# FlowEternal/multitask-hydranet

Hardware: AMD Instinct MI355X
Metric: images/sec (fwd+bwd) HydraNet @ default res, 1/2/4/8 MI355X; CPU-ref same run (higher is better)
Workload: dtype bf16; 1 GPU; full HydraNet (backbone + BiFPN + seg/det/lane heads + multitask loss), big cfg, fwd+loss+bwd; batch_per_gpu=16, global_batch=16, resolution=3x512x1024, parallelism=dp1, hipgraph=True

## Files before the change

include/hydranet_hip.h:

```cpp
#ifndef HYDRANET_HIP_H
#define HYDRANET_HIP_H

#ifdef __cplusplus
extern "C" {
#endif

typedef struct ihipStream_t* hipStream_t;


int hn_gconv_pack_diag(const float* w, void* wk, void* wd, int C, hipStream_t stream);
int hn_pack_weight(const float* w, void* wp, void* wt, int Cout, int Cin, int taps, hipStream_t stream);
int hn_pack_weight_ex(const float* w, void* wp, void* wt, int Cout, int Cin_total, int ci0, int Cin, int taps, int phase, const float* bias,
                      float* b_eff, hipStream_t stream);
int hn_phase_fold(const float* dw_eff, const float* dw1, const float* db_eff, float* dw, float* db, int K, int C0, int C1, hipStream_t stream);
int hn_pack_weights_batched(const long* jobs, int njobs, long total_blocks, const int* block_job, hipStream_t stream);
int hn_pack_small_batched(const long* jobs, const int* block_job, long total_blocks, hipStream_t stream);

int hn_conv_gemm_nt(const void* x0, const void* x1, int mode, int n_img, int H, int W, int C0, int C1, int ld0, int ld1, int up, long M,
                    const void* w, int Nout, int KP, int taps, const float* bias, int act, void* out, int out_f32, int ldc, long rpi,
                    long img_stride, float* psum, float* psq, hipStream_t stream);
int hn_nt_stat_rows(long M, int Nout);
int hn_nt_stat_tile(long M, int Nout);
int hn_direct_stat_rows(int n_img, int H, int W);
int hn_conv_gemm_nt_imgw(const void* x0, int ld0, long M, int C0, const void* w, long w_img_stride, long rows_per_image, int Nout, int KP,
// ... 14 lines not shown
                         int ld_ez, const float* ecoef, hipStream_t stream);
int hn_conv_gemm_nt_stat3(const void* x0, int ld0, long M, int C0, const void* w, int Nout, int KP, void* out, int ldc, float* psum, float* psq,
                          const void* addend, int ld_add, const void* ez, int ld_ez, const void* ey, int ld_ey, const float* ecoef,
                          hipStream_t stream);
int hn_wgrad_plan(int mode, int n_img, int H, int W, long M, int Nout, int KP, int taps, int* splits, long* rows_per_split, long* ws_bytes);
int hn_conv_gemm_tn(const void* x0, const void* x1, int mode, int n_img, int H, int W, int C0, int C1, int ld0, int ld1, int up, long M,
                    const void* dz, int ldz, int Nout, int KP, int taps, float* workspace, float* dw, hipStream_t stream);


int hn_stem_fwd(const float* x, const float* w, void* z, void* patches, int N, int H, int W, hipStream_t stream);

int hn_gconv_pack(const float* w, void* wk, void* wd, int C, int flip, hipStream_t stream);
int hn_gconv_fwd(const void* in, int ldi, const void* wk, void* out, int ldo, int N, int Hi, int Wi, int C, int stride, hipStream_t stream);
int hn_gconv_dgrad_s2(const void* dz, int ldz, const void* wd, void* dx, int ldx, int N, int Hi, int Wi, int C, hipStream_t stream);
long hn_wgrad_chunks(long pixels, long items);
int hn_gconv_wgrad(const void* x, int ldx, const void* dz, int ldz, float* part, int N, int Hi, int Wi, int C, int stride,
                   hipStream_t stream);

int hn_dw_pack(const float* w, void* wk, void* wkf, int C, hipStream_t stream);
int hn_dwconv_fwd(const void* in, int ldi, const void* wk, void* out, int ldo, int N, int H, int W, int C, hipStream_t stream);
int hn_dwconv_fwd_levels(const void* in, int ldi, const void* wk, void* out, int ldo, int N, int C, int nlev, const int* H, const int* W,
                         int row_align, int accumulate, hipStream_t stream);
long hn_dwconv_wgrad_blocks(long strips, int C);
int hn_dwconv_wgrad(const void* x, int ldx, const void* dz, int ldz, float* part, int N, int H, int W, int C, hipStream_t stream);
int hn_dwconv_wgrad_levels(const void* x, int ldx, const void* dz, int ldz, float* part, int N, int C, int nlev, const int* H, const int* W,
                           int row_align, hipStream_t stream);
long hn_dwconv_bwd_blocks(long strips, int C);
long hn_dwconv_bwd_blocks_levels(int N, int C, int nlev, const int* H, const int* W);
int hn_dwconv_bwd_levels(const void* dz, int ldz, const void* x, int ldx, const void* wf, void* dx, int lddx, float* part, int N, int C,
                         int nlev, const int* H, const int* W, int row_align, int accumulate, hipStream_t stream);

int hn_maxpool_fwd(const void* in, int ldi, void* out, int ldo, int N, int H, int W, int C, int mode, hipStream_t stream);
int hn_maxpool_bwd(const void* in, int ldi, const void* dout, int ldd, void* dx, int ldx, const float* wscale, int N, int H, int W, int C,
                   int mode, hipStream_t stream);
int hn_maxpool_bwd2(const void* in, int ldi, const void* dout, int ldd, void* dx, int ldx, const float* wscale, void* arg_ws, int N, int H,
                    int W, int C, int mode, int accumulate, hipStream_t stream);

int hn_up2_fwd(const void* in, int ldi, void* out, int ldo, int N, int H, int W, int C, hipStream_t stream);
int hn_sum2x2(const void* g, int ldg, void* out, int ldo, const float* wscale, int N, int H, int W, int C, int accumulate, hipStream_t stream);

int hn_fuse_dweights(const float* pw, int blocks, const float* praw, int nw, float eps, float* dp, hipStream_t stream);
int hn_fuse_fwd(const void* const* in, const int* ld, const int* mode, const float* w, void* out, int ldo, int N, int H, int W, int C,
                hipStream_t stream);
int hn_fuse_fwd_raw(const void* const* in, const int* ld, const int* mode, const float* praw, int nw, float eps, float* wn, void* out, int ldo,
                    int N, int H, int W, int C, hipStream_t stream);
int hn_fuse_bwd_blocks(int N, int H, int W, int C);
int hn_fuse_bwd(const void* const* in, const int* ld, const int* mode, const float* w, const void* dout, int ldd, void* g, int ldg,
                void* const* din, const int* ldin, const int* acc, float* pw, int N, int H, int W, int C, hipStream_t stream);
int hn_fuse_bwd_arg(const void* const* in, const int* ld, const int* mode, const float* w, const void* dout, int ldd, void* g, int ldg,
                    void* const* din, const int* ldin, const int* acc, float* pw, void* const* arg_out, int N, int H, int W, int C,
                    hipStream_t stream);
int hn_maxpool_bwd_from_arg(const void* arg, const void* dout, int ldd, void* dx, int ldx, const float* wscale, int N, int H, int W, int C,
                            int mode, int accumulate, hipStream_t stream);

long hn_fold_ring_rows(int H, int W);
int hn_conv3x3_dgrad_fold(const void* dz, int ldz, int Cz, int n_img, int H, int W, const void* wt, int Nout, int KP, int phase_k, int clamp,
                          void* out, int ldo, const void* yprev, int ldy, void* ring, hipStream_t stream);
int hn_conv3x3_dgrad_fold_s2d(const void* dz, int ldz, int Cz, int n_img, int H, int W, const void* wt, int Nout, int KP, int phase_k, int clamp,
                              void* out, int ldo, void* out_s2d, int ld_s2d, const void* yprev, int ldy, void* ring, hipStream_t stream);
int hn_seg_fold(const void* dvp, int ldv, int c0, void* out, int ldo, const void* yprev, int ldy, int N, int H, int W, int C, int up,
                hipStream_t stream);

int hn_space_to_depth(const float* dy, void* out, int ldo, int N, int h, int w, int k, hipStream_t stream);

int hn_space_to_depth_blocks(int N, int h, int w, int k);
int hn_space_to_depth_bf16(const void* in, int ldi, void* out, int N, int h, int w, int k, float* psum, hipStream_t stream);

int hn_conv3x3_phase(const void* x0, int mode, int n_img, int H, int W, int C0, int ld0, const void* w, int Nout, int KP, const float* bias,
                     int act, void* out, int ldc, int k, const void* addend, int ld_add, hipStream_t stream);
int hn_conv3x3_out_argmax(const void* x0, int n_img, int H, int W, int C0, int ld0, const void* w, int k, int KP, const float* bias, long* mask,
                          hipStream_t stream);
int hn_wgrad_plan_phase(int n_img, int H, int W, int Nout, int KP, int phase_span, int* splits, long* rows_per_split, long* ws_bytes);
int hn_conv_gemm_tn_phase(const void* x0, int n_img, int H, int W, int C0, int ld0, const void* dz, int ldz, int Nout, int KP, int phase_span,
                          float* workspace, float* dw, float* dbias_eff, hipStream_t stream);
int hn_conv_gemm_tn_deferred(const void* x0, const void* x1, int mode, int n_img, int H, int W, int C0, int C1, int ld0, int ld1, int up, long M,
                             const void* dz, int ldz, int Nout, int KP, int taps, float* workspace, float* dw, long* job, hipStream_t stream);
int hn_wgrad_reduce_jobs(const long* jobs, int njobs, hipStream_t stream);
long hn_gconv_wgrad_group_ws_bytes(const long* jobs, int njobs);
int hn_gconv_wgrad_group(const long* jobs, int njobs, float* workspace, hipStream_t stream);

int hn_grad_tail(const long* jobs, int njobs, hipStream_t stream);

long hn_wgrad_group_ws_bytes(const long* jobs, int njobs);
int hn_wgrad_group(const long* jobs, int njobs, float* workspace, hipStream_t stream);

int hn_conv_gemm_tn_bias(const void* x0, const void* x1, int mode, int n_img, int H, int W, int C0, int C1, int ld0, int ld1, int up, long M,
                         const void* dz, int ldz, int Nout, int KP, int taps, float* workspace, float* dw, float* dbias, hipStream_t stream);

int hn_head_grad(const float* dy, const float* y, long rpi, long img_stride, int lds, int Nout, void* dz, int ldz, long M, int sigmoid,
                 hipStream_t stream);

int hn_pack_levels(const void* const* src, const int* ld, void* dst, int ldd, int N, int C, int nlev, const int* H, const int* W, int row_align,
                   hipStream_t stream);
int hn_head_grad_levels(const float* dy, const float* y, long img_stride, int lds, int Nout, void* dz, int ldz, int N, int nlev, const int* H,
                        const int* W, int row_align, int sigmoid, hipStream_t stream);


long hn_colred_rows(long M, long align);
int hn_col_stats(const void* x, int ldx, long M, int C, long R, float* psum, float* psq, hipStream_t stream);
int hn_col_dot(const void* a, int lda, const void* b, int ldb, long M, int C, long R, float* pdot, float* psum, hipStream_t stream);
int hn_rows_reduce(const float* in, float* out, int G, int S, int C, float alpha, hipStream_t stream);
int hn_rows_reduce2(const float* in1, const float* in2, float* out1, float* out2, int rows, int G, int C, hipStream_t stream);

int hn_bn_finalize(const float* psum, const float* psq, int prows, int C, long count, const float* gamma, const float* beta, float eps,
                   float momentum, float* running_mean, float* running_var, float* scale, float* shift, float* mean, float* rstd,
                   hipStream_t stream);
// ... 193 lines not shown
```

multitask_hydranet_amd/_lib.py:

```python
from __future__ import annotations

import ctypes
import os
import re
import subprocess
from typing import Dict, List, Tuple

_PKG = os.path.dirname(os.path.abspath(__file__))
_ROOT = os.path.dirname(_PKG)
HEADER = os.path.join(_ROOT, "include", "hydranet_hip.h")
CSRC = os.path.join(_PKG, "csrc")
TUNING = os.environ.get("HN_TUNING") == "1"
AB = TUNING or os.environ.get("HN_TUNING") == "ab"


def policy(name: str, default: str) -> str:
    return os.environ.get(name, default) if AB else default

SO_PATH = os.path.join(_PKG, "libhydranet_hip_tuning.so" if TUNING else "libhydranet_hip.so")
SOURCES = ["hn_gemm.hip", "hn_norm.hip", "hn_fused.hip", "hn_stencil.hip", "hn_loss.hip", "hn_lovasz.hip", "hn_post.hip", "hn_xstage.hip", "hn_coco.hip",
           "hn_lane_encode.hip", "hn_augment.hip", "hn_jpeg.hip", "hn_jpeg_enc.hip", "hn_jpeg_huff.hip", "hn_jpeg_scan.hip", "hn_draw.hip", "hn_lane_metric.hip", "hn_png.hip", "hn_png_enc.hip"]

_ERR = {1: "bad argument", 2: "kernel launch failure", 3: "unsupported shape"}


class HipKernelError(RuntimeError):
    pass


def _ctype(decl: str):
    decl = decl.strip()
    if "*" in decl or "hipStream_t" in decl:
        return ctypes.c_void_p
    words = decl.replace("const", " ").split()
    base = words[0]
    return {"int": ctypes.c_int, "long": ctypes.c_long, "float": ctypes.c_float, "double": ctypes.c_double}[base]


TUNING_HEADER = os.path.join(_ROOT, "include", "hydranet_hip_tuning.h")


def parse_header(path: str = HEADER) -> Dict[str, Tuple[object, List[object], bool]]:
    txt = open(path).read()
    if TUNING and path == HEADER:
        txt += open(TUNING_HEADER).read()
    txt = re.sub(r"/\*.*?\*/", " ", txt, flags=re.S)
    out = {}
    for m in re.finditer(r"\b(int|long)\s+(hn_\w+)\s*\((.*?)\)\s*;", txt, flags=re.S):
        ret, name, params = m.group(1), m.group(2), m.group(3)
        plist = [p for p in (q.strip() for q in params.replace("\n", " ").split(",")) if p and p != "void"]
        args = [_ctype(p) for p in plist]
        out[name] = (ctypes.c_int if ret == "int" else ctypes.c_long, args, bool(plist) and "hipStream_t" in plist[-1])
    return out


def sources() -> List[str]:
    return [os.path.join(CSRC, s) for s in SOURCES if os.path.exists(os.path.join(CSRC, s))]


def build(force: bool = False, verbose: bool = False) -> str:
    srcs = sources()
    deps = srcs + [os.path.join(CSRC, "hn_common.h"), os.path.join(CSRC, "hn_jpeg_tables.h"), os.path.join(CSRC, "hn_jpeg_scan.h")]
    if not force and os.path.exists(SO_PATH) and all(os.path.getmtime(SO_PATH) >= os.path.getmtime(d) for d in deps):
        return SO_PATH
    hipcc = os.environ.get("HIPCC", "/opt/rocm/bin/hipcc")
    objs = []
    procs = []
    for s in srcs:
        o = os.path.join(CSRC, os.path.basename(s).replace(".hip", ".tuning.o" if TUNING else ".o"))
        objs.append(o)
        cmd = [hipcc, "--offload-arch=gfx950", "-O3", "-fPIC", "-std=c++17"] + (["-DHN_TUNING"] if TUNING else []) + ["-c", s, "-o", o]
        if verbose:
            print(" ".join(cmd))
        procs.append((cmd, subprocess.Popen(cmd, stdout=subprocess.PIPE, stderr=subprocess.STDOUT)))
# ... 57 lines not shown
```

multitask_hydranet_amd/csrc/hn_common.h:

```cpp
#pragma once
#include <hip/hip_runtime.h>
#include <stdint.h>

typedef __bf16 bf16;
typedef bf16 bf16x4 __attribute__((ext_vector_type(4)));
typedef bf16 bf16x2 __attribute__((ext_vector_type(2)));
typedef bf16 bf16x8 __attribute__((ext_vector_type(8)));
typedef short short4v __attribute__((ext_vector_type(4)));
typedef float f32x4 __attribute__((ext_vector_type(4)));
typedef unsigned int u32x4 __attribute__((ext_vector_type(4)));
typedef unsigned int u32x2 __attribute__((ext_vector_type(2)));

#define HN_OK 0
#define HN_ERR_ARG 1
#define HN_ERR_LAUNCH 2
#define HN_ERR_UNSUPPORTED 3

#define HN_CHECK_ARG(cond) do { if (!(cond)) return HN_ERR_ARG; } while (0)
#define HN_LAUNCH_CHECK() do { if (hipGetLastError() != hipSuccess) return HN_ERR_LAUNCH; return HN_OK; } while (0)

__device__ __forceinline__ float bf2f(bf16 v) { return (float)v; }
__device__ __forceinline__ bf16 f2bf(float v) { return (bf16)v; }
__device__ __forceinline__ float bfround(float v) { return (float)((bf16)v); }

// ... 59 lines not shown
        for (int k = 0; k < N; ++k) v[k] = v[k] > 0.f ? v[k] : 0.f;
    } else if (act == HN_ACT_SWISH) {
#pragma unroll
        for (int k = 0; k < N; ++k) v[k] = v[k] * sigmoidf_(v[k]);
    } else if (act == HN_ACT_ELU) {
#pragma unroll
        for (int k = 0; k < N; ++k) v[k] = v[k] > 0.f ? v[k] : (__expf(v[k]) - 1.0f);
    } else {
#pragma unroll
        for (int k = 0; k < N; ++k) v[k] = sigmoidf_(v[k]);
    }
}
template <int N>
__device__ __forceinline__ void act_bwd_n(const float (&x)[N], float (&g)[N], int act) {
    if (act == HN_ACT_NONE) return;
    if (act == HN_ACT_RELU) {
#pragma unroll
        for (int k = 0; k < N; ++k) g[k] = x[k] > 0.f ? g[k] : 0.f;
    } else if (act == HN_ACT_SWISH) {
#pragma unroll
        for (int k = 0; k < N; ++k) { const float s = sigmoidf_(x[k]); g[k] *= s * (1.f + x[k] * (1.f - s)); }
    } else if (act == HN_ACT_ELU) {
#pragma unroll
        for (int k = 0; k < N; ++k) g[k] *= x[k] > 0.f ? 1.f : __expf(x[k]);
    } else {
#pragma unroll
        for (int k = 0; k < N; ++k) { const float s = sigmoidf_(x[k]); g[k] *= s * (1.f - s); }
    }
}

__device__ __forceinline__ int xcd_remap(int hw, int nwg) {
    const int q = nwg >> 3, r = nwg & 7, x = hw & 7;
    return (x < r ? x * (q + 1) : r * (q + 1) + (x - r) * q) + (hw >> 3);
}

template <int CTRL>
__device__ __forceinline__ float dpp_mov(float v) {
    return __builtin_bit_cast(float, __builtin_amdgcn_update_dpp(0, __builtin_bit_cast(int, v), CTRL, 0xf, 0xf, false));
}
__device__ __forceinline__ float row16_sum(float v) {
    v += dpp_mov<0x128>(v);
    v += dpp_mov<0x124>(v);
    v += dpp_mov<0x122>(v);
    v += dpp_mov<0x121>(v);
    return v;
}

__device__ __forceinline__ float wave_sum(float v) {
    const int b = __builtin_bit_cast(int, row16_sum(v));
    return (__builtin_bit_cast(float, __builtin_amdgcn_readlane(b, 0)) + __builtin_bit_cast(float, __builtin_amdgcn_readlane(b, 16))) +
           (__builtin_bit_cast(float, __builtin_amdgcn_readlane(b, 32)) + __builtin_bit_cast(float, __builtin_amdgcn_readlane(b, 48)));
}

static inline int cdiv(long a, long b) { return (int)((a + b - 1) / b); }

#include <atomic>
#include <initializer_list>
static inline bool lds_optin(std::atomic<unsigned long long>& done, std::initializer_list<const void*> kernels) {
    int dev = 0;
    if (hipGetDevice(&dev) != hipSuccess || dev < 0 || dev >= 64) return false;
    const unsigned long long bit = 1ull << dev;
    if (done.load(std::memory_order_acquire) & bit) return true;
    for (const void* k : kernels)
        if (hipFuncSetAttribute(k, hipFuncAttributeMaxDynamicSharedMemorySize, 160 * 1024) != hipSuccess) return false;
    done.fetch_or(bit, std::memory_order_release);
    return true;
}
```

multitask_hydranet_amd/csrc/hn_stencil.hip:

```cpp
#include "hn_common.h"

__global__ __launch_bounds__(256) void stem_fwd_kernel(const float* x, const float* w, bf16* z, bf16* patches, int N, int H, int W) {
    const int bidx = xcd_remap(blockIdx.x, gridDim.x);
    __shared__ float sw[27][32];
    for (int i = threadIdx.x; i < 27 * 32; i += 256) {
        const int co = i & 31, t = i >> 5;
        sw[t][co] = w[co * 27 + t];
    }
    __syncthreads();
    const int Ho = H >> 1, Wo = W >> 1, Wp = (Wo + 1) >> 1;
    const long total = (long)N * Ho * Wp;
    const long idx = (long)bidx * 256 + threadIdx.x;
    if (idx >= total) return;
    const int ox = (int)(idx % Wp) * 2;
    const long t1 = idx / Wp;
    const int oy = (int)(t1 % Ho);
    const long n = t1 / Ho;
    const bool two = ox + 1 < Wo;
    float acc[2][32];
#pragma unroll
    for (int c = 0; c < 32; ++c) { acc[0][c] = 0.f; acc[1][c] = 0.f; }
    __shared__ __attribute__((aligned(16))) bf16 sp[2][256][36];
    bf16* prow = patches ? sp[0][threadIdx.x] : nullptr;
    constexpr int PH = 256 * 36;
// ... 819 lines not shown
                    for (int j = 0; j < 3; ++j) {
                        const bf16x4 zq = win[(rq + rr) % 3][j];
#pragma unroll
                        for (int k = 0; k < 4; ++k) {
                            const float zf = bf2f(zq[k]);
                            if (HAS_DX) da[k] = fmaf(zf, wr[rr * 3 + j][k], da[k]);
                            acc[8 - (rr * 3 + j)][k] = fmaf(xv[k], zf, acc[8 - (rr * 3 + j)][k]);
                        }
                    }
                if (HAS_DX && oy0 + r < H && ox0 + col < W) {
                    bf16* dst = dx + (row0 + (long)(oy0 + r) * W + ox0 + col) * lddx + cq * 4;
                    bf16x4 v;
                    if (accumulate) {
                        const bf16x4 prev = ld4(dst);
#pragma unroll
                        for (int k = 0; k < 4; ++k) v[k] = f2bf(da[k] + bf2f(prev[k]));
                    } else {
#pragma unroll
                        for (int k = 0; k < 4; ++k) v[k] = f2bf(da[k]);
                    }
                    *reinterpret_cast<bf16x4*>(dst) = v;
                }
            }
        }
    }
    __syncthreads();
    float* red = reinterpret_cast<float*>(smem);
    if (active) {
#pragma unroll
        for (int tq = 0; tq < 9; ++tq)
#pragma unroll
            for (int k = 0; k < 4; ++k) red[(colh * C4 + cq) * 37 + tq * 4 + k] = acc[tq][k];
    }
    __syncthreads();
    float* dst = part + (long)bidx * C * 9;
    for (int o = tid; o < C4 * 36; o += 256) {
        const int g = o / 36, v = o - g * 36;
        float sum = 0.f;
#pragma unroll
        for (int c2 = 0; c2 < 8; ++c2) sum += red[(c2 * C4 + g) * 37 + v];
        dst[(long)(g * 4 + (v & 3)) * 9 + (v >> 2)] = sum;
    }
}

__global__ void dw_pack_kernel(const float* w, bf16* wk, bf16* wkf, int C) {
    const int idx = blockIdx.x * blockDim.x + threadIdx.x;
    if (idx >= 9 * C) return;
    const int c = idx % C, tap = idx / C;
    const bf16 v = f2bf(w[c * 9 + tap]);
    wk[idx] = v;
    if (wkf) wkf[(8 - tap) * C + c] = v;
}

__device__ __forceinline__ void pool_window(const bf16* in, int ldi, long n, int H, int W, int oy, int ox, int c, int mode, float* best,
                                            int* arg) {
#pragma unroll
    for (int k = 0; k < 8; ++k) { best[k] = -INFINITY; arg[k] = -1; }
    const int off = mode ? -1 : 0;
#pragma unroll
    for (int ky = 0; ky < 3; ++ky)
#pragma unroll
        for (int kx = 0; kx < 3; ++kx) {
            const int iy = 2 * oy + ky + off, ix = 2 * ox + kx + off;
            const bool inside = iy >= 0 && iy < H && ix >= 0 && ix < W;
            if (!inside && mode) continue;
            bf16x8 v = inside ? ld8(in + ((n * H + iy) * (long)W + ix) * ldi + c) : zero8();
#pragma unroll
            for (int k = 0; k < 8; ++k) {
                const float f = bf2f(v[k]);
                if (f > best[k]) { best[k] = f; arg[k] = inside ? ky * 3 + kx : 9; }
            }
        }
}

__global__ __launch_bounds__(256) void maxpool_fwd_kernel(const bf16* in, int ldi, bf16* out, int ldo, int N, int H, int W, int C,
                                                          int mode) {
    const int bidx = xcd_remap(blockIdx.x, gridDim.x);
    const int C8 = C >> 3, Ho = H >> 1, Wo = W >> 1;
    const long total = (long)N * Ho * Wo * C8;
    for (long idx = (long)bidx * 256 + threadIdx.x; idx < total; idx += (long)gridDim.x * 256) {
        const int cg = (int)(idx % C8);
        long t = idx / C8;
        const int ox = (int)(t % Wo);
        t /= Wo;
        const int oy = (int)(t % Ho);
        const long n = t / Ho;
        float best[8];
        int arg[8];
        pool_window(in, ldi, n, H, W, oy, ox, cg * 8, mode, best, arg);
        bf16x8 v;
#pragma unroll
        for (int k = 0; k < 8; ++k) v[k] = f2bf(best[k]);
        st8(out + ((n * Ho + oy) * (long)Wo + ox) * ldo + cg * 8, v);
    }
}

__global__ __launch_bounds__(256) void maxpool_bwd_kernel(const bf16* in, int ldi, const bf16* dout, int ldd, bf16* dx, int ldx,
                                                          const float* wscale, int N, int H, int W, int C, int mode) {
    const int bidx = xcd_remap(blockIdx.x, gridDim.x);
    const int C8 = C >> 3, Ho = H >> 1, Wo = W >> 1;
    const long total = (long)N * H * W * C8;
    const float ws = wscale ? *wscale : 1.0f;
    const int off = mode ? -1 : 0;
    for (long idx = (long)bidx * 256 + threadIdx.x; idx < total; idx += (long)gridDim.x * 256) {
        const int cg = (int)(idx % C8);
        long t = idx / C8;
        const int ix = (int)(t % W);
        t /= W;
        const int iy = (int)(t % H);
        const long n = t / H;
        float acc[8];
#pragma unroll
        for (int k = 0; k < 8; ++k) acc[k] = 0.f;
        for (int oy = (iy - off - 2 + 1) >> 1; 2 * oy + off <= iy; ++oy) {
            if (oy < 0 || oy >= Ho) continue;
            for (int ox = (ix - off - 2 + 1) >> 1; 2 * ox + off <= ix; ++ox) {
                if (ox < 0 || ox >= Wo) continue;
                float best[8];
                int arg[8];
                pool_window(in, ldi, n, H, W, oy, ox, cg * 8, mode, best, arg);
                const int mine = (iy - 2 * oy - off) * 3 + (ix - 2 * ox - off);
                const bf16x8 g = ld8(dout + ((n * Ho + oy) * (long)Wo + ox) * ldd + cg * 8);
#pragma unroll
                for (int k = 0; k < 8; ++k)
                    if (arg[k] == mine) acc[k] += bf2f(g[k]);
            }
        }
// ... 979 lines not shown
```

multitask_hydranet_amd/model.py:

```python
from __future__ import annotations

import contextlib
import itertools
import math
import sys
import weakref
from typing import Dict, List, Optional, Sequence

import numpy as np
import torch
import torch.nn as nn

from . import ops as K
from .ops import ACT_ELU, ACT_NONE, ACT_RELU, ACT_SIGMOID, ACT_SWISH

BN_STD = dict(eps=1e-5, momentum=0.1)
BN_FPN = dict(eps=1e-3, momentum=0.01)


def regnet_stages(initial_width, slope, quantized_param, network_depth, bottleneck_ratio, group_width):
    u = initial_width + slope * np.arange(network_depth)
    s = np.round(np.log(u / initial_width) / np.log(quantized_param))
    q = 8 * np.round(initial_width * np.power(quantized_param, s) / 8)
    widths, depths = np.unique(q.astype(np.int32), return_counts=True)
# ... 386 lines not shown
        x = x.contiguous().float()
        t = self._cba(x, p + "stem.conv", p + "stem.bn", BN_STD, kind="stem", act=ACT_RELU)
        feats = []
        P = self._idx
        for k, d in enumerate(self.depths):
            group = None
            names = [f"{p}stage_{k}.blocks.block_{i}.{c}" for i in range(d)
                     for c in ("conv_block_1.0.weight", "conv_block_2.0.weight", "conv_block_3.0.weight", "shortcut.0.weight", "se.1.weight",
                               "se.1.bias", "se.3.weight", "se.3.bias")]
            names = [nm for nm in names if nm in P]
            if (K.DEFER_WGRAD and self.training and torch.is_grad_enabled() and t.requires_grad and t.is_cuda and (self.se_ratio is not None) and
                    all(P[nm].requires_grad for nm in names)):
                group = K.WgradGroup()
                t = K.DeferredGrads.apply(t, group, *[P[nm] for nm in names])
            i = 0
            while i < d:
                q = f"{p}stage_{k}.blocks.block_{i}."
                if i > 0 and self.training and not (torch.is_grad_enabled() and t.requires_grad) and self._xstage_shape_ok(q, t):
                    while i < d:
                        j1 = min(d, i + 16)
                        params = []
                        for j in range(i, j1):
                            params += self._xblock_params(f"{p}stage_{k}.blocks.block_{j}.")
                        with torch.no_grad():
                            t = K.xstage_forward_raw(t, params, BN_STD["eps"], BN_STD["momentum"])["out"][j1 - i - 1]
                        i = j1
                    break
                if i > 0 and i < d and self._xstage_run(q, t, group):
                    while i < d:
                        j1 = min(d, i + 16)
                        params = []
                        for j in range(i, j1):
                            params += self._xblock_params(f"{p}stage_{k}.blocks.block_{j}.")
                        t = K.xstage_apply(t, group, BN_STD["eps"], BN_STD["momentum"], params)
                        i = j1
                    break
                t = self._xblock(q, t, self.backbone_stride if i == 0 else 1, group)
                i += 1
            last = k == len(self.depths) - 1
            if last and tail is not None and K.DEFER_WGRAD and self.training and torch.is_grad_enabled() and t.requires_grad and t.is_cuda:
                t = K.DeferredGrads.apply(t, tail[0], *tail[1])
                tail[2] = True
            al, slot = K.share(t, ext[k] + (0 if last else 1))
            feats.append((al[:ext[k]], slot))
            if not last:
                t = al[-1]
        return feats

    def _sepconv(self, name, x, act=ACT_NONE):
        P = self._idx
        d = K.DwConv.apply(x, P[name + ".depthwise_conv.conv.weight"])
        return self._cba(d, name + ".pointwise_conv.conv", name + ".bn", BN_FPN, act=act)

    def _fusew(self, name):
        return self._idx[name]

    CELL_IN_COUNTS = (1, 2, 2, 2, 2)

    def _cell_shared(self, p, inputs, first, ext):
        red = lambda nm, src, i: self._cba(src[0][i], p + nm + ".0.conv", p + nm + ".1", BN_FPN, act=ACT_NONE, slot=src[1])
        sh = K.share
        if first:
            if len(inputs) == 4:
                p3, p4, p5 = inputs[-3:]
                p6_in = K.MaxPool.apply(red("p5_to_p6", p5, 2), 0)
            else:
                p3, p4, p5, p6r = inputs[-4:]
                p6_in = red("p6_down_channel", p6r, 0)
            (p6a, p6b, p6c), s6 = sh(p6_in, 3)
            p7_in = K.MaxPool.apply(p6c, 0)
            p3a, s3 = red("p3_down_channel", p3, 0), None
            (p4a, p4b), s4a, s4b = (red("p4_down_channel", p4, 0), red("p4_down_channel_2", p4, 1)), None, None
            (p5a, p5b), s5a, s5b = (red("p5_down_channel", p5, 0), red("p5_down_channel_2", p5, 1)), None, None
        else:
            (p3a,), s3 = inputs[0]
            (p4a, p4b), s4a = inputs[1]
            (p5a, p5b), s5a = inputs[2]
            (p6a, p6b), s6 = inputs[3]
            s4b, s5b = s4a, s5a
        if first:
            (p7a, p7b), s7 = sh(p7_in, 2)
        else:
            (p7a, p7b), s7 = inputs[4]
        F = K.Fuse.apply
        w = lambda nm: self._fusew(p + nm)
        (u6a, u6b), t6 = sh(self._sepconv(p + "conv6_up", F(w("p6_w1"), 1, 2, 0, p6a, p7a, None, (s6, s7, None))), 2)
        (u5a, u5b), t5 = sh(self._sepconv(p + "conv5_up", F(w("p5_w1"), 1, 2, 0, p5a, u6a, None, (s5a, t6, None))), 2)
        (u4a, u4b), t4 = sh(self._sepconv(p + "conv4_up", F(w("p4_w1"), 1, 2, 0, p4a, u5a, None, (s4a, t5, None))), 2)
        o3, q3 = sh(self._sepconv(p + "conv3_up", F(w("p3_w1"), 1, 2, 0, p3a, u4a, None, (s3, t4, None))), 1 + ext[0])
        o4, q4 = sh(self._sepconv(p + "conv4_down", F(w("p4_w2"), 1, 1, 3, p4b, u4b, o3[0], (s4b, t4, q3))), 1 + ext[1])
        o5, q5 = sh(self._sepconv(p + "conv5_down", F(w("p5_w2"), 1, 1, 3, p5b, u5b, o4[0], (s5b, t5, q4))), 1 + ext[2])
        o6, q6 = sh(self._sepconv(p + "conv6_down", F(w("p6_w2"), 1, 1, 3, p6b, u6b, o5[0], (s6, t6, q5))), 1 + ext[3])
        o7, q7 = sh(self._sepconv(p + "conv7_down", F(w("p7_w2"), 1, 3, 0, p7b, o6[0], None, (s7, q6, None))), ext[4])
        return [(o3[1:], q3), (o4[1:], q4), (o5[1:], q5), (o6[1:], q6), (o7, q7)]

    def first_cell_counts(self):
        n = len(self.depths)
        cnt = [0] * n
        if n == 4:
            cnt[-3:] = [1, 2, 3]
        else:
            cnt[-4:] = [1, 2, 2, 1]
        return cnt

    def _cell(self, p, inputs, first):
        ins = [((t, t, t), None) for t in inputs] if first else [K.share(t, c) for t, c in zip(inputs, self.CELL_IN_COUNTS)]
        return tuple(a[0] for a, _ in self._cell_shared(p, ins, first, (1, 1, 1, 1, 1)))

    def _neck_shared(self, feats, head_counts):
        x = list(feats)
        for k in range(self.fpn_cell_repeats):
            last = k == self.fpn_cell_repeats - 1
            x = self._cell_shared(f"neck.bifpn.{k}.", x, k == 0, head_counts if last else self.CELL_IN_COUNTS)
        return [aliases for aliases, _ in x]

    def _neck(self, feats):
        return [a[0] for a in self._neck_shared([((t, t, t), None) for t in feats], (1, 1, 1, 1, 1))]

    def _seg(self, feats_seg, want_mask=False):
        P = self._idx
        n = len(feats_seg)
        x = feats_seg[-1]
        p = "segheader.decoder."
        fuse = self.seg_fuse_elu_bwd
        s2d = False
        slot = None
        for i in range(n):
            x = K.SegConv.apply(x, None, P[f"{p}{2 * i}.conv.conv.weight"], P[f"{p}{2 * i}.conv.conv.bias"], 0, ACT_ELU, False,
                                fuse and i > 0, fuse, slot)
            slot = None
            skip = feats_seg[n - 2 - i] if i < n - 1 else None
            wgt = P[f"{p}{2 * i + 1}.conv.conv.weight"]
            if K.seg_up_phase_ok(x, skip, wgt):
                s2d = bool(fuse and i == n - 1 and self.seg_phase_output and self.training and x.requires_grad
                           and not want_mask and K.seg_s2d_handover_ok(x, skip, wgt))
                slot = K.GradSlot() if (fuse and not s2d and self.training and x.requires_grad) else None
                x = K.SegConvUp.apply(x, skip, wgt, P[f"{p}{2 * i + 1}.conv.conv.bias"], fuse, fuse, s2d, slot)
            else:
                x = K.SegConv.apply(x, skip, wgt, P[f"{p}{2 * i + 1}.conv.conv.bias"], 1, ACT_ELU, False, fuse, fuse)
        last = 2 * n
        if want_mask and self.seg_phase_output and K.seg_out_argmax_ok(x, P[f"{p}{last}.conv.weight"]):
            return K.seg_out_argmax(x, P[f"{p}{last}.conv.weight"], P[f"{p}{last}.conv.bias"])
        if self.seg_phase_output:
            slot = K.GradSlot() if (x.requires_grad and self.training) else None
            y = K.SegOutUp.apply(x, P[f"{p}{last}.conv.weight"], P[f"{p}{last}.conv.bias"], fuse, slot, s2d)
            out = y.permute(0, 3, 1, 2)
# ... 288 lines not shown
```

multitask_hydranet_amd/ops/neck.py:

```python
from __future__ import annotations

import ctypes
import os
from typing import Optional, Sequence, Tuple

import torch

from .._lib import lib, policy
from .core import *
from .backbone import *


def k_dwconv(x, wk, out=None):
    n, h, w, c = x.shape
    if out is None:
        out = new_act(n, h, w, c, x.device)
    lib().call("hn_dwconv_fwd", ptr(x), ld(x), ptr(wk), ptr(out), ld(out), n, h, w, c)
    return out


def k_dwconv_wgrad(x, dz):
    n, h, w, c = x.shape
    chunks = lib().query("hn_dwconv_wgrad_blocks", n * h * ((w + 3) // 4), c)
    part = torch.empty((chunks, c * 9), device=x.device, dtype=F32)
# ... 137 lines not shown
        return out

    @staticmethod
    def backward(ctx, dout):
        praw, w = ctx.saved_tensors[0], ctx.saved_tensors[1]
        rest = list(ctx.saved_tensors[2:])
        ins = [rest.pop(0) if m else None for m in ctx.modes]
        dpraw, dins = fuse_backward(praw, w, ins, ctx.modes, ctx.slots, ctx.queue, ctx.pref, dense(dout))
        return dpraw, None, None, None, dins[0], dins[1], dins[2], None


def fuse_backward(praw, w, ins, modes, slots, queue, pref, dout):
    n, h, wd, ch = dout.shape
    dev = dout.device
    g = new_act(n, h, wd, ch, dev)
    dst, accum = [None] * 3, [0] * 3
    for i, m in enumerate(modes):
        if not m:
            continue
        sl = slots[i]
        if sl is not None and sl.buf is not None:
            dst[i], accum[i] = sl.buf, 1
        else:
            dst[i] = new_act(*ins[i].shape, dev)
            if sl is not None:
                sl.buf = dst[i]
    ap, al, am = _fuse_args(ins, modes)
    inside = (1, 2) if FUSE_SUM2X2 else (1,)
    dp_ = (ctypes.c_void_p * 3)(*[ptr(dst[i]) if modes[i] in inside else None for i in range(3)])
    dl = (ctypes.c_int * 3)(*[ld(dst[i]) if modes[i] in inside else 0 for i in range(3)])
    da = (ctypes.c_int * 3)(*accum)
    blocks = lib().query("hn_fuse_bwd_blocks", n, h, wd, ch)
    pw = torch.empty((blocks, 3), device=dev, dtype=F32)
    args = [torch.empty((n * h * wd * ch,), device=dev, dtype=torch.uint8) if (m == 3 and FUSE_ARG) else None for m in modes]
    aa = (ctypes.c_void_p * 3)(*[ptr(t) for t in args])
    lib().call("hn_fuse_bwd_arg", ctypes.addressof(ap), ctypes.addressof(al), ctypes.addressof(am), ptr(w), ptr(dout), ld(dout), ptr(g),
               ld(g), ctypes.addressof(dp_), ctypes.addressof(dl), ctypes.addressof(da), ptr(pw), ctypes.addressof(aa), n, h, wd, ch)
    if queue is not None:
        dpraw = queue.add_fuse(pref, pw, blocks, 1e-4)
    else:
        dpraw = torch.empty_like(praw)
        lib().call("hn_fuse_dweights", ptr(pw), blocks, ptr(praw), praw.numel(), 1e-4, ptr(dpraw))
    for i, m in enumerate(modes):
        if m == 2 and not FUSE_SUM2X2:
            lib().call("hn_sum2x2", ptr(g), ld(g), ptr(dst[i]), ld(dst[i]), ptr(w[i]), n, h // 2, wd // 2, ch, accum[i])
        elif m == 3 and not FUSE_ARG:
            k_maxpool_bwd(ins[i], g, 0, wscale=w[i], into=dst[i], accumulate=bool(accum[i]))
        elif m == 3:
            lib().call("hn_maxpool_bwd_from_arg", ptr(args[i]), ptr(g), ld(g), ptr(dst[i]), ld(dst[i]), ptr(w[i]), n, 2 * h, 2 * wd, ch, 0,
                       accum[i])
    return dpraw, [None if (slots[i] is not None or not modes[i]) else dst[i] for i in range(3)]


__all__ = [n for n in dir() if not n.startswith("__")]
```

Before: 981.5 images/sec.

## Fuse small BiFPN nodes into a single weighted-fuse, depthwise, pointwise and BN-stats kernel

Adds a fused HIP kernel for BiFPN nodes at small spatial sizes (N*H*W up to 2048, W up to 64). In one launch it computes the normalized weighted fusion with swish, the depthwise 3x3 conv from LDS, the pointwise conv via MFMA, and the per-band BN partial sums. A new autograd Function reuses the existing backward pieces. The aim is to cut launch count and intermediate global round-trips on the tiny low-resolution BiFPN levels, which are launch-bound. The cost is a large LDS footprint per block, and each band does only one 64-pixel MFMA tile, so parallelism is limited.

```diff
diff --git a/include/hydranet_hip.h b/include/hydranet_hip.h
--- a/include/hydranet_hip.h
+++ b/include/hydranet_hip.h
@@ -90,6 +90,12 @@
                     hipStream_t stream);
 int hn_maxpool_bwd_from_arg(const void* arg, const void* dout, int ldd, void* dx, int ldx, const float* wscale, int N, int H, int W, int C,
                             int mode, int accumulate, hipStream_t stream);
+
+int hn_bifpn_node_ok(int N, int H, int W, int C, const int* modes);
+int hn_bifpn_node_blocks(int N, int H, int W);
+int hn_bifpn_node_fwd(const void* const* in, const int* ld, const int* mode, const float* praw, int nw, float eps, float* wn,
+                      const void* wdw, const void* wpw, int KP, const float* bias, void* f, int ldf, void* d, int ldd, void* z, int ldz,
+                      float* psum, float* psq, int N, int H, int W, int C, hipStream_t stream);
 
 long hn_fold_ring_rows(int H, int W);
 int hn_conv3x3_dgrad_fold(const void* dz, int ldz, int Cz, int n_img, int H, int W, const void* wt, int Nout, int KP, int phase_k, int clamp,
diff --git a/multitask_hydranet_amd/_lib.py b/multitask_hydranet_amd/_lib.py
--- a/multitask_hydranet_amd/_lib.py
+++ b/multitask_hydranet_amd/_lib.py
@@ -19,7 +19,7 @@
 
 SO_PATH = os.path.join(_PKG, "libhydranet_hip_tuning.so" if TUNING else "libhydranet_hip.so")
 SOURCES = ["hn_gemm.hip", "hn_norm.hip", "hn_fused.hip", "hn_stencil.hip", "hn_loss.hip", "hn_lovasz.hip", "hn_post.hip", "hn_xstage.hip", "hn_coco.hip",
-           "hn_lane_encode.hip", "hn_augment.hip", "hn_jpeg.hip", "hn_jpeg_enc.hip", "hn_jpeg_huff.hip", "hn_jpeg_scan.hip", "hn_draw.hip", "hn_lane_metric.hip", "hn_png.hip", "hn_png_enc.hip"]
+           "hn_lane_encode.hip", "hn_augment.hip", "hn_jpeg.hip", "hn_jpeg_enc.hip", "hn_jpeg_huff.hip", "hn_jpeg_scan.hip", "hn_draw.hip", "hn_lane_metric.hip", "hn_png.hip", "hn_png_enc.hip", "hn_bifpn_node.hip"]
 
 _ERR = {1: "bad argument", 2: "kernel launch failure", 3: "unsupported shape"}
 
diff --git a/multitask_hydranet_amd/csrc/hn_bifpn_node.hip b/multitask_hydranet_amd/csrc/hn_bifpn_node.hip
--- /dev/null
+++ b/multitask_hydranet_amd/csrc/hn_bifpn_node.hip
@@ -0,0 +1,212 @@
+#include "hn_common.h"
+
+struct BifpnNode {
+    const bf16* in[3]; int ld[3]; int mode[3];
+    const float* praw; int nw; float eps; float* wn;
+    const bf16* wdw;
+    const bf16* wpw; int KP;
+    const float* bias;
+    bf16 *f, *d, *z; int ldf, ldd, ldz;
+    float *psum, *psq;
+    int N, H, W, C, rb, bands;
+};
+
+__device__ __forceinline__ int dswz(int row, int pc, int kp8) { return (row * kp8 + (pc ^ (row & 7 & (kp8 - 1)))) * 16; }
+
+#define NODE_THREADS 1024
+__global__ __launch_bounds__(NODE_THREADS) void bifpn_node_fwd_kernel(const BifpnNode p) {
+    extern __shared__ __attribute__((aligned(16))) char smem[];
+    const int tid = threadIdx.x, lane = tid & 63, wave = __builtin_amdgcn_readfirstlane(tid >> 6);
+    const int cw = wave & 3, pw = wave >> 2;
+    const int lid = xcd_remap(blockIdx.x, gridDim.x);
+    const int n = lid / p.bands, y0 = (lid % p.bands) * p.rb;
+    const int C8 = p.C >> 3, KP8 = p.KP >> 3, H = p.H, W = p.W;
+    const int nrow = min(p.rb, H - y0), npix = nrow * W;
+    const int hrows = p.rb + 2;
+    bf16* sF = reinterpret_cast<bf16*>(smem);
+    char* sD = smem + (size_t)hrows * W * p.C * 2;
+    float* red = reinterpret_cast<float*>(sD + 64 * p.KP * 2);
+    bf16* sWd = reinterpret_cast<bf16*>(red + 4 * p.C * 2);
+
+    float wv[3];
+    {
+        float sum = 0.f;
+#pragma unroll
+        for (int i = 0; i < 3; ++i) { wv[i] = i < p.nw ? fmaxf(p.praw[i], 0.f) : 0.f; sum += wv[i]; }
+#pragma unroll
+        for (int i = 0; i < 3; ++i) wv[i] = wv[i] / (sum + p.eps);
+        if (lid == 0 && tid < 3) p.wn[tid] = wv[tid];
+    }
+
+    for (int i = tid; i < 64 * KP8; i += NODE_THREADS) *reinterpret_cast<bf16x8*>(sD + i * 16) = zero8();
+    for (int i = tid; i < 9 * C8; i += NODE_THREADS) st8(sWd + i * 8, ld8(p.wdw + i * 8));
+
+    for (int idx = tid; idx < hrows * W * C8; idx += NODE_THREADS) {
+        const int cg = idx % C8;
+        int t = idx / C8;
+        const int x = t % W, hr = t / W, y = y0 - 1 + hr;
+        bf16x8 o = zero8();
+        if (y >= 0 && y < H && hr <= nrow + 1) {
+            float acc[8];
+#pragma unroll
+            for (int k = 0; k < 8; ++k) acc[k] = 0.f;
+#pragma unroll
+            for (int i = 0; i < 3; ++i) {
+                if (!p.mode[i]) continue;
+                float v[8];
+                if (p.mode[i] == 1) {
+                    const bf16x8 s = ld8(p.in[i] + (((long)n * H + y) * W + x) * p.ld[i] + cg * 8);
+#pragma unroll
+                    for (int k = 0; k < 8; ++k) v[k] = bf2f(s[k]);
+                } else if (p.mode[i] == 2) {
+                    const bf16x8 s = ld8(p.in[i] + (((long)n * (H >> 1) + (y >> 1)) * (W >> 1) + (x >> 1)) * p.ld[i] + cg * 8);
+#pragma unroll
+                    for (int k = 0; k < 8; ++k) v[k] = bf2f(s[k]);
+                } else {
+                    int arg[8];
+                    pool_window(p.in[i], p.ld[i], n, 2 * H, 2 * W, y, x, cg * 8, 0, v, arg);
+                }
+                const float wi = wv[i];
+#pragma unroll
+                for (int k = 0; k < 8; ++k) acc[k] = fmaf(wi, v[k], acc[k]);
+            }
+#pragma unroll
+            for (int k = 0; k < 8; ++k) o[k] = f2bf(act_fwd(acc[k], HN_ACT_SWISH));
+            if (hr >= 1 && hr <= nrow) st8(p.f + (((long)n * H + y) * W + x) * p.ldf + cg * 8, o);
+        }
+        st8(sF + ((long)hr * W + x) * p.C + cg * 8, o);
+    }
+    const int ksteps = p.KP >> 5;
+    bf16x8 wfr[2][4];
+    float pbias[2][4];
+#pragma unroll
+    for (int i = 0; i < 2; ++i) {
+        const int co = (cw * 2 + i) * 16 + (lane & 15);
+#pragma unroll
+        for (int ks = 0; ks < 4; ++ks)
+            wfr[i][ks] = (ks < ksteps && co < p.C) ? ld8(p.wpw + (long)co * p.KP + ks * 32 + (lane >> 4) * 8) : zero8();
+        const int co0 = (cw * 2 + i) * 16 + (lane >> 4) * 4;
+#pragma unroll
+        for (int r = 0; r < 4; ++r) pbias[i][r] = (p.bias && co0 + r < p.C) ? p.bias[co0 + r] : 0.f;
+    }
+
+    __syncthreads();
+
+    for (int idx = tid; idx < npix * C8; idx += NODE_THREADS) {
+        const int cg = idx % C8, pix = idx / C8;
+        const int x = pix % W, r = pix / W, y = y0 + r;
+        float acc[8];
+#pragma unroll
+        for (int k = 0; k < 8; ++k) acc[k] = 0.f;
+#pragma unroll
+        for (int ky = 0; ky < 3; ++ky) {
+            const int iy = y + ky - 1;
+            if (iy < 0 || iy >= H) continue;
+#pragma unroll
+            for (int kx = 0; kx < 3; ++kx) {
+                const int ix = x + kx - 1;
+                const bf16x8 v = (ix >= 0 && ix < W) ? ld8(sF + ((long)(r + ky) * W + ix) * p.C + cg * 8) : zero8();
+                const bf16x8 wt = ld8(sWd + (ky * 3 + kx) * p.C + cg * 8);
+#pragma unroll
+                for (int k = 0; k < 8; ++k) acc[k] = fmaf(bf2f(v[k]), bf2f(wt[k]), acc[k]);
+            }
+        }
+        bf16x8 o;
+#pragma unroll
+        for (int k = 0; k < 8; ++k) o[k] = f2bf(acc[k]);
+        st8(p.d + (((long)n * H + y) * W + x) * p.ldd + cg * 8, o);
+        *reinterpret_cast<bf16x8*>(sD + dswz(pix, cg, KP8)) = o;
+    }
+    __syncthreads();
+
+    if (cw * 32 < p.C) {
+        f32x4 acc[2];
+#pragma unroll
+        for (int i = 0; i < 2; ++i) acc[i] = (f32x4){0.f, 0.f, 0.f, 0.f};
+#pragma unroll
+        for (int ks = 0; ks < 4; ++ks) {
+            if (ks >= ksteps) break;
+            const bf16x8 b = *reinterpret_cast<const bf16x8*>(sD + dswz(pw * 16 + (lane & 15), ks * 4 + (lane >> 4), KP8));
+#pragma unroll
+            for (int i = 0; i < 2; ++i) acc[i] = __builtin_amdgcn_mfma_f32_16x16x32_bf16(wfr[i][ks], b, acc[i], 0, 0, 0);
+        }
+        const int pix = pw * 16 + (lane & 15);
+        const bool pv = pix < npix;
+#pragma unroll
+        for (int i = 0; i < 2; ++i) {
+            const int co0 = (cw * 2 + i) * 16 + (lane >> 4) * 4;
+            float s1[4], s2[4];
+            bf16x4 t;
+#pragma unroll
+            for (int r = 0; r < 4; ++r) {
+                t[r] = f2bf(acc[i][r] + pbias[i][r]);
+                const float q = pv ? bf2f(t[r]) : 0.f;
+                s1[r] = row16_sum(q);
+                s2[r] = row16_sum(q * q);
+            }
+            if (pv && co0 < p.C) {
+                const int x = pix % W, y = y0 + pix / W;
+                *reinterpret_cast<bf16x4*>(p.z + (((long)n * H + y) * W + x) * p.ldz + co0) = t;
+            }
+            if ((lane & 15) == 0 && co0 < p.C) {
+#pragma unroll
+                for (int r = 0; r < 4; ++r) { red[(pw * p.C + co0 + r) * 2] = s1[r]; red[(pw * p.C + co0 + r) * 2 + 1] = s2[r]; }
+            }
+        }
+    }
+    __syncthreads();
+    if (tid < p.C) {
+        float a = 0.f, b = 0.f;
+#pragma unroll
+        for (int j = 0; j < 4; ++j) { a += red[(j * p.C + tid) * 2]; b += red[(j * p.C + tid) * 2 + 1]; }
+        p.psum[(long)lid * p.C + tid] = a;
+        p.psq[(long)lid * p.C + tid] = b;
+    }
+}
+
+#define HN_BIFPN_NODE_MAX_ROWS 2048
+
+static inline int node_rb(int H, int W) { const int rb = 64 / W; return rb < H ? rb : H; }
+static inline size_t node_lds(int H, int W, int C) {
+    return (size_t)(node_rb(H, W) + 2) * W * C * 2 + (size_t)64 * ((C + 31) & ~31) * 2 + (size_t)4 * C * 2 * 4 + (size_t)9 * C * 2;
+}
+
+static bool node_shape_ok(int N, int H, int W, int C, const int* modes) {
+    if (!modes || N < 1 || H < 1 || W < 1 || W > 64 || C < 8 || C > 128 || (C & 7)) return false;
+    if (modes[0] != 1) return false;
+    for (int i = 1; i < 3; ++i) {
+        if (modes[i] < 0 || modes[i] > 3) return false;
+        if (modes[i] == 2 && ((H | W) & 1)) return false;
+    }
+    return node_lds(H, W, C) <= 64 * 1024 && (long)N * H * W * 128 < (1L << 31);
+}
+
+extern "C" int hn_bifpn_node_ok(int N, int H, int W, int C, const int* modes) {
+    return node_shape_ok(N, H, W, C, modes) && (long)N * H * W <= HN_BIFPN_NODE_MAX_ROWS ? 1 : 0;
+}
+
+extern "C" int hn_bifpn_node_blocks(int N, int H, int W) {
+    if (N < 1 || H < 1 || W < 1 || W > 64) return 0;
+    const int rb = node_rb(H, W);
+    return N * ((H + rb - 1) / rb);
+}
+
+extern "C" int hn_bifpn_node_fwd(const void* const* in, const int* ld, const int* mode, const float* praw, int nw, float eps, float* wn,
+                                 const void* wdw, const void* wpw, int KP, const float* bias, void* f, int ldf, void* d, int ldd, void* z,
+                                 int ldz, float* psum, float* psq, int N, int H, int W, int C, hipStream_t st) {
+    HN_CHECK_ARG(in && ld && mode && praw && wn && nw >= 1 && nw <= 3 && wdw && wpw && f && d && z && psum && psq);
+    if (!node_shape_ok(N, H, W, C, mode)) return HN_ERR_UNSUPPORTED;
+    HN_CHECK_ARG(KP == ((C + 31) & ~31) && !(ldf & 7) && !(ldd & 7) && !(ldz & 7) && ldf >= C && ldd >= C && ldz >= C);
+    BifpnNode p;
+    for (int i = 0; i < 3; ++i) {
+        HN_CHECK_ARG(mode[i] == 0 || (in[i] && !(ld[i] & 7) && ld[i] >= C));
+        p.in[i] = (const bf16*)in[i]; p.ld[i] = ld[i]; p.mode[i] = mode[i];
+    }
+    p.praw = praw; p.nw = nw; p.eps = eps; p.wn = wn;
+    p.wdw = (const bf16*)wdw; p.wpw = (const bf16*)wpw; p.KP = KP; p.bias = bias;
+    p.f = (bf16*)f; p.d = (bf16*)d; p.z = (bf16*)z; p.ldf = ldf; p.ldd = ldd; p.ldz = ldz;
+    p.psum = psum; p.psq = psq;
+    p.N = N; p.H = H; p.W = W; p.C = C; p.rb = node_rb(H, W); p.bands = (H + p.rb - 1) / p.rb;
+    hipLaunchKernelGGL(bifpn_node_fwd_kernel, dim3(N * p.bands), dim3(NODE_THREADS), node_lds(H, W, C), st, p);
+    HN_LAUNCH_CHECK();
+}
diff --git a/multitask_hydranet_amd/csrc/hn_common.h b/multitask_hydranet_amd/csrc/hn_common.h
--- a/multitask_hydranet_amd/csrc/hn_common.h
+++ b/multitask_hydranet_amd/csrc/hn_common.h
@@ -135,6 +135,27 @@
            (__builtin_bit_cast(float, __builtin_amdgcn_readlane(b, 32)) + __builtin_bit_cast(float, __builtin_amdgcn_readlane(b, 48)));
 }
 
+__device__ __forceinline__ void pool_window(const bf16* in, int ldi, long n, int H, int W, int oy, int ox, int c, int mode, float* best,
+                                            int* arg) {
+#pragma unroll
+    for (int k = 0; k < 8; ++k) { best[k] = -INFINITY; arg[k] = -1; }
+    const int off = mode ? -1 : 0;
+#pragma unroll
+    for (int ky = 0; ky < 3; ++ky)
+#pragma unroll
+        for (int kx = 0; kx < 3; ++kx) {
+            const int iy = 2 * oy + ky + off, ix = 2 * ox + kx + off;
+            const bool inside = iy >= 0 && iy < H && ix >= 0 && ix < W;
+            if (!inside && mode) continue;
+            bf16x8 v = inside ? ld8(in + ((n * H + iy) * (long)W + ix) * ldi + c) : zero8();
+#pragma unroll
+            for (int k = 0; k < 8; ++k) {
+                const float f = bf2f(v[k]);
+                if (f > best[k]) { best[k] = f; arg[k] = inside ? ky * 3 + kx : 9; }
+            }
+        }
+}
+
 static inline int cdiv(long a, long b) { return (int)((a + b - 1) / b); }
 
 #include <atomic>
diff --git a/multitask_hydranet_amd/csrc/hn_stencil.hip b/multitask_hydranet_amd/csrc/hn_stencil.hip
--- a/multitask_hydranet_amd/csrc/hn_stencil.hip
+++ b/multitask_hydranet_amd/csrc/hn_stencil.hip
@@ -895,27 +895,6 @@
     if (wkf) wkf[(8 - tap) * C + c] = v;
 }
 
-__device__ __forceinline__ void pool_window(const bf16* in, int ldi, long n, int H, int W, int oy, int ox, int c, int mode, float* best,
-                                            int* arg) {
-#pragma unroll
-    for (int k = 0; k < 8; ++k) { best[k] = -INFINITY; arg[k] = -1; }
-    const int off = mode ? -1 : 0;
-#pragma unroll
-    for (int ky = 0; ky < 3; ++ky)
-#pragma unroll
-        for (int kx = 0; kx < 3; ++kx) {
-            const int iy = 2 * oy + ky + off, ix = 2 * ox + kx + off;
-            const bool inside = iy >= 0 && iy < H && ix >= 0 && ix < W;
-            if (!inside && mode) continue;
-            bf16x8 v = inside ? ld8(in + ((n * H + iy) * (long)W + ix) * ldi + c) : zero8();
-#pragma unroll
-            for (int k = 0; k < 8; ++k) {
-                const float f = bf2f(v[k]);
-                if (f > best[k]) { best[k] = f; arg[k] = inside ? ky * 3 + kx : 9; }
-            }
-        }
-}
-
 __global__ __launch_bounds__(256) void maxpool_fwd_kernel(const bf16* in, int ldi, bf16* out, int ldo, int N, int H, int W, int C,
                                                           int mode) {
     const int bidx = xcd_remap(blockIdx.x, gridDim.x);
diff --git a/multitask_hydranet_amd/model.py b/multitask_hydranet_amd/model.py
--- a/multitask_hydranet_amd/model.py
+++ b/multitask_hydranet_amd/model.py
@@ -462,6 +462,14 @@
         d = K.DwConv.apply(x, P[name + ".depthwise_conv.conv.weight"])
         return self._cba(d, name + ".pointwise_conv.conv", name + ".bn", BN_FPN, act=act)
 
+    def _node(self, name, praw, m0, m1, m2, a, b, c, slots):
+        P = self._idx
+        pw = P[name + ".pointwise_conv.conv.weight"]
+        if self.training and a.is_cuda and pw.shape[0] == pw.shape[1] == a.shape[3] and K.bifpn_node_ok(a, (m0, m1, m2)):
+            return K.BifpnNode.apply(praw, m0, m1, m2, a, b, c, slots, P[name + ".depthwise_conv.conv.weight"], pw,
+                                     P.get(name + ".pointwise_conv.conv.bias"), *self._bn(name + ".bn"), BN_FPN["eps"], BN_FPN["momentum"])
+        return self._sepconv(name, K.Fuse.apply(praw, m0, m1, m2, a, b, c, slots))
+
     def _fusew(self, name):
         return self._idx[name]
 
@@ -492,16 +500,16 @@
             (p7a, p7b), s7 = sh(p7_in, 2)
         else:
             (p7a, p7b), s7 = inputs[4]
-        F = K.Fuse.apply
+        node = self._node
         w = lambda nm: self._fusew(p + nm)
-        (u6a, u6b), t6 = sh(self._sepconv(p + "conv6_up", F(w("p6_w1"), 1, 2, 0, p6a, p7a, None, (s6, s7, None))), 2)
-        (u5a, u5b), t5 = sh(self._sepconv(p + "conv5_up", F(w("p5_w1"), 1, 2, 0, p5a, u6a, None, (s5a, t6, None))), 2)
-        (u4a, u4b), t4 = sh(self._sepconv(p + "conv4_up", F(w("p4_w1"), 1, 2, 0, p4a, u5a, None, (s4a, t5, None))), 2)
-        o3, q3 = sh(self._sepconv(p + "conv3_up", F(w("p3_w1"), 1, 2, 0, p3a, u4a, None, (s3, t4, None))), 1 + ext[0])
-        o4, q4 = sh(self._sepconv(p + "conv4_down", F(w("p4_w2"), 1, 1, 3, p4b, u4b, o3[0], (s4b, t4, q3))), 1 + ext[1])
-        o5, q5 = sh(self._sepconv(p + "conv5_down", F(w("p5_w2"), 1, 1, 3, p5b, u5b, o4[0], (s5b, t5, q4))), 1 + ext[2])
-        o6, q6 = sh(self._sepconv(p + "conv6_down", F(w("p6_w2"), 1, 1, 3, p6b, u6b, o5[0], (s6, t6, q5))), 1 + ext[3])
-        o7, q7 = sh(self._sepconv(p + "conv7_down", F(w("p7_w2"), 1, 3, 0, p7b, o6[0], None, (s7, q6, None))), ext[4])
+        (u6a, u6b), t6 = sh(node(p + "conv6_up", w("p6_w1"), 1, 2, 0, p6a, p7a, None, (s6, s7, None)), 2)
+        (u5a, u5b), t5 = sh(node(p + "conv5_up", w("p5_w1"), 1, 2, 0, p5a, u6a, None, (s5a, t6, None)), 2)
+        (u4a, u4b), t4 = sh(node(p + "conv4_up", w("p4_w1"), 1, 2, 0, p4a, u5a, None, (s4a, t5, None)), 2)
+        o3, q3 = sh(node(p + "conv3_up", w("p3_w1"), 1, 2, 0, p3a, u4a, None, (s3, t4, None)), 1 + ext[0])
+        o4, q4 = sh(node(p + "conv4_down", w("p4_w2"), 1, 1, 3, p4b, u4b, o3[0], (s4b, t4, q3)), 1 + ext[1])
+        o5, q5 = sh(node(p + "conv5_down", w("p5_w2"), 1, 1, 3, p5b, u5b, o4[0], (s5b, t5, q4)), 1 + ext[2])
+        o6, q6 = sh(node(p + "conv6_down", w("p6_w2"), 1, 1, 3, p6b, u6b, o5[0], (s6, t6, q5)), 1 + ext[3])
+        o7, q7 = sh(node(p + "conv7_down", w("p7_w2"), 1, 3, 0, p7b, o6[0], None, (s7, q6, None)), ext[4])
         return [(o3[1:], q3), (o4[1:], q4), (o5[1:], q5), (o6[1:], q6), (o7, q7)]
 
     def first_cell_counts(self):
diff --git a/multitask_hydranet_amd/ops/neck.py b/multitask_hydranet_amd/ops/neck.py
--- a/multitask_hydranet_amd/ops/neck.py
+++ b/multitask_hydranet_amd/ops/neck.py
@@ -213,4 +213,69 @@
     return dpraw, [None if (slots[i] is not None or not modes[i]) else dst[i] for i in range(3)]
 
 
+BIFPN_NODE = policy("HN_BIFPN_NODE", "1") != "0"
+
+
+def bifpn_node_ok(x, modes):
+    n, h, w, c = x.shape
+    return bool(BIFPN_NODE and FUSED_BN and lib().query("hn_bifpn_node_ok", n, h, w, c, ctypes.addressof((ctypes.c_int * 3)(*modes))))
+
+
+def k_bifpn_node_fwd(praw, ins, modes, wk, wp, bias):
+    n, h, wd, ch = ins[0].shape
+    dev = ins[0].device
+    w = torch.empty((3,), device=dev, dtype=F32)
+    f, d, z = (new_act(n, h, wd, ch, dev) for _ in range(3))
+    blocks = lib().query("hn_bifpn_node_blocks", n, h, wd)
+    psum = torch.empty((blocks, ch), device=dev, dtype=F32)
+    psq = torch.empty((blocks, ch), device=dev, dtype=F32)
+    ap, al, am = _fuse_args(ins, modes)
+    lib().call("hn_bifpn_node_fwd", ctypes.addressof(ap), ctypes.addressof(al), ctypes.addressof(am), ptr(praw), praw.numel(), 1e-4, ptr(w),
+               ptr(wk), ptr(wp), kp32(ch), ptr(bias), ptr(f), ld(f), ptr(d), ld(d), ptr(z), ld(z), ptr(psum), ptr(psq), n, h, wd, ch)
+    return w, f, d, z, psum, psq
+
+
+class BifpnNode(torch.autograd.Function):
+
+    @staticmethod
+    def forward(ctx, praw, m0, m1, m2, a, b, c, slots, dw_weight, pw_weight, pw_bias, gamma, beta, rm, rv, nbt, eps, momentum):
+        ins, modes = [a, b, c], [m0, m1, m2]
+        wk, wf = pack_dw_weight(dw_weight)
+        wp, wt = pack_conv_weight(pw_weight)
+        w, f, d, z, psum, psq = k_bifpn_node_fwd(praw, ins, modes, wk, wp, pw_bias)
+        n, h, wd, ch = z.shape
+        ctx.count = n * h * wd
+        out, coef, _, _ = k_bn_apply_fused(z, psum, psq, ctx.count, gamma, beta, eps, momentum, rm, rv, ACT_NONE, training=True)
+        if nbt is not None:
+            nbt.add_(1)
+        ctx.modes = modes
+        ctx.slots = slots if slots is not None else (None, None, None)
+        q = cur_queue()
+        ctx.q_fuse = q if praw.requires_grad else None
+        ctx.q_dw = q if dw_weight.requires_grad else None
+        ctx.q_pw = q if pw_weight.requires_grad else None
+        ctx.refs = (praw, dw_weight, pw_weight)
+        ctx.has_bias = pw_bias is not None
+        ctx.save_for_backward(praw, w, f, d, z, coef, wf, wt, *[t for t in ins if t is not None])
+        return out
+
+    @staticmethod
+    def backward(ctx, dout):
+        praw, w, f, d, z, coef, wf, wt = ctx.saved_tensors[:8]
+        rest = list(ctx.saved_tensors[8:])
+        ins = [rest.pop(0) if m else None for m in ctx.modes]
+        pref, dwref, pwref = ctx.refs
+        n, h, wd, ch = z.shape
+        dbias = torch.empty((ch,), device=z.device, dtype=F32) if ctx.has_bias else None
+        dz, dgamma, dbeta, _ = bn_backward_fused(dense(dout), z, None, coef, ACT_NONE, ctx.count, zero_c=dbias)
+        dd, _, _ = k_gemm_nt(dz, None, 0, (n, h, wd), wt, ch, kp32(ch), 1)
+        if ctx.q_pw is not None:
+            dpw = ctx.q_pw.add_gemm(pwref, d, dz, 0, (n, h, wd), ch, ch)
+        else:
+            dpw = k_gemm_tn(d, None, 0, (n, h, wd), dz, ch, kp32(ch), 1, ch)
+        df, ddw = k_dwconv_bwd(dd, f, wf, queue=ctx.q_dw, weight=dwref)
+        dpraw, dins = fuse_backward(praw, w, ins, ctx.modes, ctx.slots, ctx.q_fuse, pref, df)
+        return (dpraw, None, None, None, dins[0], dins[1], dins[2], None, ddw, dpw, dbias, dgamma, dbeta) + (None,) * 5
+
+
 __all__ = [n for n in dir() if not n.startswith("__")]
```

Result: no change. 983.6 images/sec (median of 6 runs) (+0.2%).
